# dsshim0125/s2p

Measured on AMD Instinct MI355X. Metric: G+D train-step images/sec at 84x84 bs=64/GPU, higher is better.
Workload: dtype bf16; 1 GPU; configs[2]: full G+D train step (hinge GAN + feature matching + VGG19 perceptual + L1, Adam x2), 84x84 cheetah, netG=s2p, netD=multiscale(2); global_batch=64, per_gpu_batch=64, parallelism=dp1, hip_graph=True, graph_segments=1, streams=overlapped, vgg_weights=seeded stand-in (ImageNet weights unobtainable offline)

## Files before the change

### include/s2p_hip.h

```cpp
#ifndef S2P_HIP_H
#define S2P_HIP_H
#include <stddef.h>
#include <stdint.h>

#ifdef __cplusplus
extern "C" {
#endif
#pragma GCC visibility push(default)

#define S2P_VERSION 125

enum { S2P_F32 = 0, S2P_BF16 = 1 };
enum { S2P_ACT_NONE = 0, S2P_ACT_RELU = 1, S2P_ACT_LRELU = 2, S2P_ACT_TANH = 3, S2P_ACT_SWISH = 4 };
enum { S2P_EPI_STORE = 0,
       S2P_EPI_ADD = 1,
       S2P_EPI_MUL_ACTGRAD = 2   };

typedef struct {
  int32_t dtype;
  int32_t N, H, W, Cin, x_pitch;
  int32_t Ho, Wo, Cout, y_pitch;
  int32_t KH, KW, stride, pad;
  int32_t transposed;
  int32_t reflect;
  int32_t groups;
  int32_t x_gstride, y_gstride;
  int32_t cin_real;
} s2p_conv_desc;

int s2p_version(void);
const char* s2p_last_error(void);

int s2p_conv2d_fwd(const s2p_conv_desc* d, const void* x, const void* w_fwd, const float* bias,
                   const void* aux, void* y, int act, float slope, int epi, void* stream);
int s2p_conv2d_dgrad(const s2p_conv_desc* d, const void* dy, const void* w_bwd,
                     const void* aux, const void* aux2, void* dx, int epi, int aux_act, float slope,
                     void* stream);
size_t s2p_conv2d_fwd_workspace(const s2p_conv_desc* d, int epi);
int s2p_conv2d_fwd_ws(const s2p_conv_desc* d, const void* x, const void* w_fwd, const float* bias,
                      const void* aux, void* y, int act, float slope, int epi, void* workspace,
                      size_t workspace_bytes, void* stream);
size_t s2p_conv2d_dgrad_workspace(const s2p_conv_desc* d);
int s2p_conv2d_dgrad_ws(const s2p_conv_desc* d, const void* dy, const void* w_bwd,
                        const void* aux, const void* aux2, void* dx, int epi, int aux_act, float slope,
                        void* workspace, size_t workspace_bytes, void* stream);
int s2p_conv2d_fwd_mat(const s2p_conv_desc* d, const void* x, const void* w_fwd, const float* bias, const void* aux,
                       void* y, int epi, const void* gb_img, int gb_pitch, const float* gb_st, int gb_st_pitch,
                       int act, float slope, float eps, void* y_mat, int y_mat_pitch, float* stats, void* workspace,
                       size_t workspace_bytes, void* stream);
int s2p_conv2d_dgrad_mat(const s2p_conv_desc* d, const void* dy, const void* w_bwd, void* d_mid, const void* aux, const void* xn,
                         int xn_pitch, const float* stats, const void* gb_img, int gb_pitch, const float* gb_st,
                         int gb_st_pitch, int act, float slope, float eps, float* sums, void* dxn, int dxn_pitch,
                         void* dgb_img, int dgb_pitch, float* dgb_st, int dgb_st_pitch, const void* res, int res_pitch,
                         void* workspace, size_t workspace_bytes, void* stream);
int s2p_conv2d_mat_is_fused(const s2p_conv_desc* d, int dgrad, int has_gb);
int s2p_conv2d_wgrad(const s2p_conv_desc* d, const void* x, const void* dy, float* dw, float* db,
                     int cin_real, int cout_real, int64_t dw_gstride, int splitk, void* stream);
size_t s2p_conv2d_wgrad_workspace(const s2p_conv_desc* d, int cin_real, int cout_real);
int s2p_conv2d_wgrad_ws(const s2p_conv_desc* d, const void* x, const void* dy, float* dw, float* db,
                        int cin_real, int cout_real, int64_t dw_gstride, int splitk, void* workspace,
                        size_t workspace_bytes, void* stream);
size_t s2p_conv2d_wgrad_det_workspace(const s2p_conv_desc* d, int cin_real, int cout_real, int splitk);
typedef struct { const void* x; const void* dy; float* dw; float* db; } s2p_wgrad_job;
size_t s2p_conv2d_wgrad_batched_workspace(const s2p_conv_desc* d, int n_jobs, int cin_real, int cout_real);
int s2p_conv2d_wgrad_batched(const s2p_conv_desc* d, const s2p_wgrad_job* jobs, int n_jobs, int cin_real,
                             int cout_real, void* workspace, size_t workspace_bytes, void* stream);
int s2p_reflect_pad_bwd(int dtype, const void* dxp, int N, int H, int W, int C, int pad, void* dx,
                        void* stream);
int s2p_channel_sum(int dtype, const void* dy, int64_t pixels, int C, int pitch, float* db,
                    void* stream);
size_t s2p_channel_sum_workspace(int64_t pixels, int C);
int s2p_channel_sum_ws(int dtype, const void* dy, int64_t pixels, int C, int pitch, float* db, void* workspace,
                       size_t workspace_bytes, void* stream);

int64_t s2p_in_stats_floats(int N, int HW, int C);
int s2p_in_stats(int dtype, const void* x, int N, int HW, int C, int pitch, float eps,
                 float* stats, void* stream);
int s2p_in_apply_fwd(int dtype, const void* x, int N, int HW, int C, int pitch,
                     const float* stats, const void* gb_img, int gb_pitch,
                     const float* gb_st, int gb_st_pitch, int act, float slope, float eps,
                     void* y, int y_pitch, void* stream);
int s2p_in_norm_fwd(int dtype, const void* x, int N, int HW, int C, int pitch, const void* gb_img, int gb_pitch,
                    const float* gb_st, int gb_st_pitch, int act, float slope, float eps, void* y, int y_pitch,
                    float* stats, void* stream);
int64_t s2p_in_bwd_sums_floats(int N, int HW, int C);
int s2p_in_bwd_reduce(int dtype, const void* da, int da_pitch, const void* x, int N, int HW, int C,
                      int pitch, const float* stats, const void* gb_img, int gb_pitch,
                      const float* gb_st, int gb_st_pitch, int act, float slope, float eps,
// ... 121 lines not shown
```

### s2p_amd/_lib.py

```python
import ctypes
import os
import subprocess

import torch

_HERE = os.path.dirname(os.path.abspath(__file__))
_SO = os.path.join(_HERE, "csrc", "libs2p_hip.so")

F32, BF16 = 0, 1
ACT_NONE, ACT_RELU, ACT_LRELU, ACT_TANH, ACT_SWISH = 0, 1, 2, 3, 4
EPI_STORE, EPI_ADD, EPI_MUL_ACTGRAD = 0, 1, 2

c_int, c_float, c_void_p, c_int64 = ctypes.c_int, ctypes.c_float, ctypes.c_void_p, ctypes.c_int64


class ConvDesc(ctypes.Structure):
    _fields_ = [(n, ctypes.c_int32) for n in (
        "dtype", "N", "H", "W", "Cin", "x_pitch", "Ho", "Wo", "Cout", "y_pitch",
        "KH", "KW", "stride", "pad", "transposed", "reflect", "groups", "x_gstride", "y_gstride", "cin_real")]


class L1Job(ctypes.Structure):
    _fields_ = [("a", c_void_p), ("b", c_void_p), ("grad_a", c_void_p), ("count", c_int64), ("scale", c_float),
                ("loss_out", c_void_p)]


class WgradJob(ctypes.Structure):
    _fields_ = [("x", c_void_p), ("dy", c_void_p), ("dw", c_void_p), ("db", c_void_p)]


class PackJob(ctypes.Structure):
    _fields_ = [("src", c_void_p), ("dst_fwd", c_void_p), ("dst_bwd", c_void_p),
                ("R", ctypes.c_int32), ("T", ctypes.c_int32), ("C", ctypes.c_int32),
                ("Cpad", ctypes.c_int32), ("Rrow", ctypes.c_int32), ("r_off", ctypes.c_int32),
                ("dtype", ctypes.c_int32)]


class SnJob(ctypes.Structure):
    _fields_ = [("w", c_void_p), ("u", c_void_p), ("v", c_void_p), ("sigma", c_void_p), ("ws", c_void_p), ("grad", c_void_p),
                ("R", ctypes.c_int32), ("K", ctypes.c_int32)]


_P = c_void_p
_DESC = ctypes.POINTER(ConvDesc)
SIGNATURES = {
    "s2p_version": [],
    "s2p_last_error": [],
    "s2p_conv2d_fwd": [_DESC, _P, _P, _P, _P, _P, c_int, c_float, c_int, _P],
    "s2p_conv2d_dgrad": [_DESC, _P, _P, _P, _P, _P, c_int, c_int, c_float, _P],
    "s2p_conv2d_fwd_workspace": [_DESC, c_int],
    "s2p_conv2d_fwd_ws": [_DESC, _P, _P, _P, _P, _P, c_int, c_float, c_int, _P, ctypes.c_size_t, _P],
    "s2p_conv2d_fwd_mat": [_DESC, _P, _P, _P, _P, _P, c_int, _P, c_int, _P, c_int, c_int, c_float, c_float, _P, c_int, _P, _P,
                           ctypes.c_size_t, _P],
    "s2p_conv2d_dgrad_mat": [_DESC, _P, _P, _P, _P, _P, c_int, _P, _P, c_int, _P, c_int, c_int, c_float, c_float, _P, _P, c_int, _P, c_int,
                             _P, c_int, _P, c_int, _P, ctypes.c_size_t, _P],
    "s2p_conv2d_mat_is_fused": [_DESC, c_int, c_int],
    "s2p_conv2d_dgrad_workspace": [_DESC],
    "s2p_conv2d_dgrad_ws": [_DESC, _P, _P, _P, _P, _P, c_int, c_int, c_float, _P, ctypes.c_size_t, _P],
    "s2p_conv2d_wgrad": [_DESC, _P, _P, _P, _P, c_int, c_int, c_int64, c_int, _P],
    "s2p_conv2d_wgrad_workspace": [_DESC, c_int, c_int],
    "s2p_conv2d_wgrad_det_workspace": [_DESC, c_int, c_int, c_int],
    "s2p_channel_sum_workspace": [c_int64, c_int],
    "s2p_channel_sum_ws": [c_int, _P, c_int64, c_int, c_int, _P, _P, ctypes.c_size_t, _P],
    "s2p_conv2d_wgrad_ws": [_DESC, _P, _P, _P, _P, c_int, c_int, c_int64, c_int, _P, ctypes.c_size_t, _P],
    "s2p_conv2d_wgrad_batched_workspace": [_DESC, c_int, c_int, c_int],
    "s2p_conv2d_wgrad_batched": [_DESC, ctypes.POINTER(WgradJob), c_int, c_int, c_int, _P, ctypes.c_size_t, _P],
    "s2p_reflect_pad_bwd": [c_int, _P, c_int, c_int, c_int, c_int, c_int, _P, _P],
    "s2p_channel_sum": [c_int, _P, c_int64, c_int, c_int, _P, _P],
    "s2p_in_stats": [c_int, _P, c_int, c_int, c_int, c_int, c_float, _P, _P],
    "s2p_in_apply_fwd": [c_int, _P, c_int, c_int, c_int, c_int, _P, _P, c_int, _P, c_int, c_int, c_float,
                         c_float, _P, c_int, _P],
    "s2p_in_norm_fwd": [c_int, _P, c_int, c_int, c_int, c_int, _P, c_int, _P, c_int, c_int, c_float, c_float, _P, c_int,
                        _P, _P],
    "s2p_in_bwd_reduce": [c_int, _P, c_int, _P, c_int, c_int, c_int, c_int, _P, _P, c_int, _P, c_int, c_int,
                          c_float, c_float, _P, _P],
    "s2p_in_bwd_apply": [c_int, _P, c_int, _P, c_int, c_int, c_int, c_int, _P, _P, c_int, _P, c_int, c_int,
                         c_float, c_float, _P, _P, c_int, _P, c_int, _P, c_int, _P],
    "s2p_in_norm_bwd": [c_int, _P, c_int, _P, c_int, c_int, c_int, c_int, _P, _P, c_int, _P, c_int, c_int,
                        c_float, c_float, _P, _P, c_int, _P, c_int, _P, c_int, _P],
    "s2p_in_norm_bwd_res": [c_int, _P, c_int, _P, c_int, c_int, c_int, c_int, _P, _P, c_int, _P, c_int, c_int,
                            c_float, c_float, _P, _P, c_int, _P, c_int, _P, c_int, _P, c_int, _P],
    "s2p_in_stats_floats": [c_int, c_int, c_int],
    "s2p_in_bwd_sums_floats": [c_int, c_int, c_int],
    "s2p_linear_fwd": [_P, c_int, c_int, c_int, _P, c_int, _P, c_int, c_int, c_float, _P, c_int, c_int, _P],
    "s2p_linear_bwd_workspace": [c_int, c_int, c_int],
    "s2p_linear_bwd": [_P, c_int, _P, c_int, _P, c_int, c_int, c_int, c_int, c_int, _P, c_int, c_int, c_float, _P, c_int, _P, _P,
                       c_int, _P, ctypes.c_size_t, _P],
    "s2p_gauss_head_fwd": [_P, c_int, c_int, c_int, _P, c_int, _P, c_int, _P, c_int, _P, c_int, _P, c_int, _P],
    "s2p_gauss_head_bwd": [_P, c_int, c_int, c_int, _P, c_int, _P, c_int, _P, c_int, _P, c_int, _P, c_int, _P, c_int, _P],
# ... 99 lines not shown
```

### s2p_amd/csrc/conv_igemm.hip

```cpp
#include "s2p_common.h"
#include "conv_plane.h"
#include "conv_planeg.h"
#include <type_traits>
#include <vector>

#define MAX_TAPS 64

constexpr int PHASE_TAPS = 16, MAX_PHASES = 4;
struct GatherArgs {
  const void* x; const void* w; const float* bias; const void* aux; const void* aux2; void* y;
  int M, Hi, Wi, Qh, Qw;
  int Cin, x_pitch, x_gstride;
  int Cout, Cst, y_pitch, y_gstride;
  int Ho, Wo;
  int istride, ostride, oy0, ox0;
  int T, Ktot, w_row;
  long long w_gstride;
  int reflect, act, epi, gact;
  float slope, gslope;
  int npix_tiles, nco_tiles;
  int halo_lo, halo_hi;
  int diag;
  int splitk, ksteps;
  float* part; int psplit, psteps, part_m;
  void* ws; size_t ws_bytes;
  size_t* plan; const PlaneMat* mat; int* mat_done;
  unsigned x_bytes, w_bytes;
  int tap[MAX_TAPS];
  int nphase, phase_fast;
  struct Phase { int Qh, Qw, M, oy0, ox0, T, Ktot, npix_tiles; int tap[PHASE_TAPS]; } ph[MAX_PHASES];
};

template <typename T> struct Mma;
template <> struct Mma<__bf16> { static constexpr int BK = 32; };
template <> struct Mma<float> { static constexpr int BK = 16; };
// ... 688 lines not shown
          if (aux2) x2.set(e, to_f32(aux2[go + e]));
        }
      }
#pragma unroll
      for (int e = 0; e < 8; ++e) {
        const float xv = x.get(e);
        const float f = g_tanh ? 1.f - xv * xv : (xv > 0.f ? 1.f : gneg);
        wv[e] = epi_add ? c.get(e) + xv : (c.get(e) + x2.get(e)) * f;
      }
      c.pack(wv);
    }
    if (full) *(u32x4*)(y + go) = c.raw;
    else for (int e = 0; e < 8; ++e) if (co0 + e < a.Cst) y[go + e] = from_f32<T>(c.get(e));
  }
}

struct ConvSwitches {
  int no_dma = s2p_env_set("S2P_NO_LDS_DMA");
  int diag = s2p_env_int("S2P_DIAG", 0);
  int no_halo = s2p_env_set("S2P_NO_HALO");
  int no_split = s2p_env_set("S2P_NO_CONV_SPLITK");
  int split_min_steps = s2p_env_int("S2P_SPLIT_MIN_STEPS", 16);
  int split_max_wg = s2p_env_int("S2P_SPLIT_MAX_WG", 160);
  int no_plane = s2p_env_set("S2P_NO_PLANE");
  int halo_extra_lds = s2p_env_int("S2P_HALO_EXTRA_LDS", 0);
  int no_static_taps = s2p_env_set("S2P_NO_STATIC_TAPS");
  int halo_pipe = s2p_env_set("S2P_NO_HALO_PIPE") ? 0 : 1;
  int no_merge = s2p_env_set("S2P_NO_PHASE_MERGE") || s2p_env_set("S2P_NO_LDS_DMA");
  int no_thin_cin = s2p_env_set("S2P_NO_THIN_CIN");
  static bool no_planeg() { return S2P_DIAG_SWITCH(0); }
  static bool no_planeg_3x3() { return S2P_DIAG_SWITCH(2); }
  static bool no_thin4() { return S2P_DIAG_SWITCH(3); }
  static bool no_phase_fast() { return S2P_DIAG_SWITCH(10); }
};
static const ConvSwitches& conv_switches() { static const ConvSwitches sw; return sw; }

static int conv_split_plan(int nwg, int nk) {
  const int min_steps = conv_switches().split_min_steps, max_wg = conv_switches().split_max_wg;
  if (nwg > max_wg || nk < 2 * min_steps) return 1;
  int S = 384 / nwg;
  if (S > nk / min_steps) S = nk / min_steps;
  if (S > 16) S = 16;
  return S < 2 ? 1 : S;
}

template <int NPOS_CAP, bool DBUF, int TS = 0, bool PIPE = false>
__global__ __launch_bounds__(256, 2) void conv_halo_kernel(const GatherArgs a) {
  typedef __bf16 T;
  constexpr int BCO = 128, BPIX = 128, WPIX = 2, TCO = 2, TPIX = 2;
  constexpr int BK = 64, RS = 128;
  constexpr int WSTAGE = BCO * RS;
  constexpr int HALO = (NPOS_CAP + 1) * RS;
  constexpr int ERS = BCO * 2 + 16;
  constexpr int EPI = BPIX * ERS;
  constexpr int NHB = DBUF ? 2 : 1;
  constexpr int MAIN0 = NHB * HALO + 2 * WSTAGE + 1024;
  constexpr int MAIN = MAIN0 > EPI ? MAIN0 : EPI;
  __shared__ __attribute__((aligned(1024))) char smem[MAIN + BPIX * 4];
  int* rowoff = (int*)(smem + MAIN);
  char* hbase = smem;
  char* wbase = smem + NHB * HALO;
  char* zrow = smem + NHB * HALO + 2 * WSTAGE;
  unsigned long long tl0 = 0, tl1 = 0, tl2 = 0;
  if (S2P_DIAGV(a) == 9) tl0 = __builtin_amdgcn_s_memrealtime();

  const int tid = threadIdx.x;
// ... 361 lines not shown
#pragma unroll
      for (int s = 0; s < 4; ++s)
#pragma unroll
        for (int i = 0; i < TCO; ++i)
#pragma unroll
          for (int j = 0; j < TPIX; ++j)
            acc[i][j] = __builtin_amdgcn_mfma_f32_32x32x16_bf16(af[s][i], bf[s][j], acc[i][j], 0, 0, 0);
    }
    __syncthreads();
    tap = ntap;
    tw_cur = tw_next; tw_next = tw_next2;
    if (nslab_i != slab) {
      slab = nslab_i;
      if (!DBUF && slab < nslab) {
        issue_halo(0, slab * BK);
        __syncthreads();
      }
    }
  }
  (void)nk;
  if (S2P_DIAGV(a) == 8) {
    const unsigned long long c1 = __builtin_amdgcn_s_memtime(), r1 = __builtin_amdgcn_s_memrealtime();
    if (tid == 0 && g == 0) {
      unsigned long long* o = (unsigned long long*)a.y + (size_t)blockIdx.x * 2;
      o[0] = c1 - st_c0; o[1] = r1 - st_r0;
    }
    if (acc[0][0][0] == 12345.678f) ((float*)a.y)[7] = acc[1][1][3] + acc[0][1][2] + acc[1][0][1];
    return;
  }
  if (S2P_DIAGV(a) == 4) { if (acc[0][0][0] == 12345.678f) ((float*)a.y)[0] = acc[1][1][3] + acc[0][1][2] + acc[1][0][1]; return; }
  conv_epilogue<T, BCO, BPIX, TCO, TPIX>(a, acc, smem, rowoff, g, co_base, wco0, wpix0, r, h, tid);
}

enum class ConvPath { Thin, Thin4, ThinCin, ThinRows, Plane, PlaneG, Halo, SplitK, Dma, Fast, Phases, Generic };
enum class HaloKind { S9_176_PIPE, S9_176, S9_320, R_176, R_320 };

struct ConvOperands {
  const void* x; const void* w; const float* bias; const void* aux; const void* aux2; void* y;
  int act; float slope; int epi, gact; float gslope;
};
struct NormWant { bool any, gb, bwd; };
struct ScratchAvail { bool any; size_t bytes; };
static const ScratchAvail SCRATCH_UNLIMITED{true, ~(size_t)0};
struct Scratch { void* ws; size_t bytes; };

struct GatherChoice {
  ConvPath path = ConvPath::Generic;
  bool fused = false;
  size_t ws_bytes = 0;
  int bco = 128;
  HaloKind halo = HaloKind::R_320;
  PlaneArgs plane;
  PlaneGArgs planeg;
};
struct GatherItem { GatherArgs a; GatherChoice c; };
struct ConvPlan {
  ConvPath path = ConvPath::Generic;
  bool fused = false;
  size_t ws_bytes = 0;
  int cout_pad = 0;
  std::vector<GatherItem> items;
  void add(const GatherItem& it) {
    if (items.empty()) path = it.c.path;
    if (it.c.ws_bytes > ws_bytes) ws_bytes = it.c.ws_bytes;
    items.push_back(it);
    fused = items.size() == 1 && it.c.fused;
  }
};

template <typename P>
static void copy_conv_fields(P& p, const GatherArgs& a) {
  p.x = a.x; p.w = a.w; p.bias = a.bias; p.aux = a.aux; p.aux2 = a.aux2; p.y = a.y;
  p.Cin = a.Cin; p.x_pitch = a.x_pitch; p.x_gstride = a.x_gstride;
  p.Cout = a.Cout; p.Cst = a.Cst; p.y_pitch = a.y_pitch; p.y_gstride = a.y_gstride;
  p.w_row = a.w_row; p.w_gstride = a.w_gstride;
  p.act = a.act; p.epi = a.epi; p.gact = a.gact; p.slope = a.slope; p.gslope = a.gslope;
  p.x_bytes = a.x_bytes; p.w_bytes = a.w_bytes;
}
template <typename P>
static void copy_norm(P& p, const PlaneMat& m) {
  p.xn = m.xn; p.xn_pitch = m.xn_pitch; p.dgb = m.dgb; p.dgb_pitch = m.dgb_pitch;
  p.dgbst = m.dgbst; p.dgbst_pitch = m.dgbst_pitch; p.res = m.res; p.res_pitch = m.res_pitch;
  p.y2 = m.y2; p.y2_pitch = m.y2_pitch; p.gb = m.gb; p.gb_pitch = m.gb_pitch;
  p.gbst = m.gbst; p.gbst_pitch = m.gbst_pitch; p.stats = m.stats;
  p.n_act = m.act; p.n_slope = m.slope; p.eps = m.eps;
}
// ... 121 lines not shown
  a.T = G.KH * G.KW; a.Ktot = a.T * G.Ci; a.reflect = G.reflect;
  if (a.T > MAX_TAPS) S2P_FAIL(-2, "conv: more than %d taps", MAX_TAPS);
  for (int ky = 0; ky < G.KH; ++ky)
    for (int kx = 0; kx < G.KW; ++kx) a.tap[ky * G.KW + kx] = pack_tap(ky - G.pad, kx - G.pad, ky * G.KW + kx);
  if (a.M > 0) P.add(plan_gather(a, bf16, G.groups, gathered_elems(G), want, sc));
  return 0;
}

static int plan_scatter_problem(const Geo& G, bool bf16, const ConvOperands& op, const NormWant& want, const ScratchAvail& sc, ConvPlan& P) {
  const ConvSwitches& sw = conv_switches();
  const int s = G.stride;
  GatherArgs base = gather_base(G, op);
  base.istride = 1; base.ostride = s;
  const long long xb = gathered_elems(G) * 2, wb = (long long)G.Co * G.w_row * 2;
  if (bf16 && !sw.no_merge && s * s <= MAX_PHASES && s > 1 && G.Ci % 64 == 0 && xb < (1ll << 31) && wb < (1ll << 31) && G.Cst > 32) {
    GatherItem it{base, {}};
    GatherArgs& a = it.a;
    a.x_bytes = (unsigned)xb; a.w_bytes = (unsigned)wb;
    a.diag = sw.diag;
    bool ok = true;
    int np = 0;
    for (int py = 0; py < s && ok; ++py)
      for (int px = 0; px < s && ok; ++px) {
        GatherArgs::Phase& ph = a.ph[np];
        ph.Qh = (G.Ho - py + s - 1) / s; ph.Qw = (G.Wo - px + s - 1) / s;
        if (ph.Qh <= 0 || ph.Qw <= 0) continue;
        ph.M = G.N * ph.Qh * ph.Qw; ph.oy0 = py; ph.ox0 = px;
        ph.T = phase_taps(G, py, px, ph.tap, PHASE_TAPS);
        if (ph.T <= 0) { ok = false; break; }
        ph.Ktot = ph.T * G.Ci;
        ph.npix_tiles = cdiv(ph.M, 128);
        ++np;
      }
    if (ok && np > 0) {
      a.nphase = np;
      it.c.path = ConvPath::Phases;
      it.c.bco = a.Cst > 64 ? 128 : 64;
      a.nco_tiles = cdiv(a.Cst, it.c.bco);
      a.phase_fast = (it.c.bco == 64 && !sw.no_phase_fast()) ? 1 : 0;
      P.add(it);
      return 0;
    }
  }
  for (int py = 0; py < s; ++py)
    for (int px = 0; px < s; ++px) {
      GatherArgs a = base;
      a.Qh = (G.Ho - py + s - 1) / s; a.Qw = (G.Wo - px + s - 1) / s;
      if (a.Qh <= 0 || a.Qw <= 0) continue;
      a.M = G.N * a.Qh * a.Qw; a.oy0 = py; a.ox0 = px;
      a.T = phase_taps(G, py, px, a.tap, MAX_TAPS);
      if (a.T < 0) S2P_FAIL(-2, "conv: more than %d taps", MAX_TAPS);
      a.Ktot = a.T * G.Ci;
      if (a.M > 0) P.add(plan_gather(a, bf16, G.groups, gathered_elems(G), want, sc));
    }
  return 0;
}

static int check_desc(const s2p_conv_desc* d, const char* who) {
  if (!d) S2P_FAIL(-1, "%s: null desc", who);
  if (d->dtype != S2P_F32 && d->dtype != S2P_BF16) S2P_FAIL(-1, "%s: bad dtype %d", who, d->dtype);
  int ce = d->dtype == S2P_F32 ? 4 : 8;
  if (d->Cin % ce || d->x_pitch % ce || d->y_pitch % ce || d->x_gstride % ce || d->y_gstride % ce)
    S2P_FAIL(-1, "%s: Cin/pitches must be multiples of %d elements (Cin=%d xp=%d yp=%d)", who, ce, d->Cin,
             d->x_pitch, d->y_pitch);
  if (d->groups < 1 || d->stride < 1 || d->KH < 1 || d->KW < 1) S2P_FAIL(-1, "%s: bad geometry", who);
  if (d->x_pitch < d->Cin || d->y_pitch < d->Cout) S2P_FAIL(-1, "%s: pitch smaller than channels", who);
// ... 79 lines not shown
    default:
      hipLaunchKernelGGL((conv_dma_kernel<BCO, 128, 2, 2>), grid, dim3(256), 0, st, a);
      S2P_CHECK_LAUNCH("conv_dma_kernel");
      return 0;
  }
}

template <typename T>
static int launch_generic(GatherArgs& a, int groups, hipStream_t st) {
  if (a.Cst > 64) return launch_cfg<T, 128, 128, 2, 2>(a, groups, st);
  if (a.Cst > 32) return launch_cfg<T, 64, 128, 2, 2>(a, groups, st);
  return launch_cfg<T, 32, 256, 1, 4>(a, groups, st);
}

static int launch_item(GatherItem& it, bool bf16, int groups, const PlaneMat* mat, void* ws, hipStream_t st) {
  if (!bf16) return launch_generic<float>(it.a, groups, st);
  switch (it.c.path) {
    case ConvPath::Plane:
      if (it.c.fused) copy_norm(it.c.plane, *mat);
      return s2p_conv_plane_launch(it.c.plane, groups, st);
    case ConvPath::PlaneG:
      if (it.c.fused) copy_norm(it.c.planeg, *mat);
      return s2p_conv_planeg_launch(it.c.planeg, groups, st);
    case ConvPath::Phases: {
      GatherArgs& a = it.a;
      int max_npt = 0;
      for (int i = 0; i < a.nphase; ++i) if (a.ph[i].npix_tiles > max_npt) max_npt = a.ph[i].npix_tiles;
      const dim3 grid = a.phase_fast ? dim3(((max_npt * a.nco_tiles + 7) / 8) * 8 * a.nphase, groups, 1) : dim3(max_npt * a.nco_tiles, groups, a.nphase);
      if (it.c.bco == 128) hipLaunchKernelGGL((conv_dma_kernel<128, 128, 2, 2>), grid, dim3(256), 0, st, a);
      else hipLaunchKernelGGL((conv_dma_kernel<64, 128, 2, 2>), grid, dim3(256), 0, st, a);
      S2P_CHECK_LAUNCH("conv_dma_kernel(phases)");
      return 0;
    }
    case ConvPath::Generic: break;
    default: return it.c.bco == 128 ? launch_bf16<128>(it.a, it.c, groups, ws, st) : launch_bf16<64>(it.a, it.c, groups, ws, st);
  }
  return launch_generic<__bf16>(it.a, groups, st);
}
static int launch_items(ConvPlan& P, bool bf16, int groups, const PlaneMat* mat, const Scratch& sc, hipStream_t st) {
  for (GatherItem& it : P.items) {
    const int rc = launch_item(it, bf16, groups, mat, sc.ws, st);
    if (rc) return rc;
  }
  return 0;
}

static int conv_fwd_impl(const s2p_conv_desc* d, const ConvOperands& op, const PlaneMat* mat, bool* fused, const Scratch& sc, void* stream) {
  S2P_CHECK_SLOPE("s2p_conv2d_fwd", op.act, op.slope);
  if (mat) S2P_CHECK_SLOPE("s2p_conv2d_fwd_mat", mat->act, mat->slope);
  ConvPlan P;
  int rc = conv_plan_fwd(d, op, NormWant{mat != nullptr, mat && mat->gb, false}, ScratchAvail{sc.ws != nullptr, sc.bytes}, P);
  if (rc) return rc;
  if (!op.x || !op.w || (!op.y && !mat)) S2P_FAIL(-1, "s2p_conv2d_fwd: null pointer");
  if (op.epi != S2P_EPI_STORE && !op.aux) S2P_FAIL(-1, "s2p_conv2d_fwd: epi needs aux");
  if (!op.y && !P.fused) S2P_FAIL(-1, "s2p_conv2d_fwd_mat: y == NULL needs the fused launch (s2p_conv2d_mat_is_fused)");
  if (fused) *fused = P.fused;
  hipStream_t st = (hipStream_t)stream;
  switch (P.path) {
    case ConvPath::Thin: return s2p_thin_fwd(d, op.x, op.w, op.bias, op.y, op.act, op.slope, st);
    case ConvPath::Thin4: return s2p_thin4_fwd(d, op.x, op.w, op.bias, op.y, op.act, op.slope, sc.ws, sc.bytes, st);
    case ConvPath::ThinCin: return s2p_thin_cin_fwd(d, op.x, op.w, op.bias, op.y, op.act, op.slope, st);
    default: return launch_items(P, d->dtype == S2P_BF16, d->groups, mat, sc, st);
  }
}

extern "C" int s2p_conv2d_fwd(const s2p_conv_desc* d, const void* x, const void* w_fwd, const float* bias,
// ... 62 lines not shown
                                    int xn_pitch, const float* stats, const void* gb_img, int gb_pitch, const float* gb_st,
                                    int gb_st_pitch, int act, float slope, float eps, float* sums, void* dxn, int dxn_pitch,
                                    void* dgb_img, int dgb_pitch, float* dgb_st, int dgb_st_pitch, const void* res, int res_pitch,
                                    void* workspace, size_t workspace_bytes, void* stream) {
  if (!d || !xn || !stats || !dxn) S2P_FAIL(-1, "s2p_conv2d_dgrad_mat: null pointer");
  if (act != S2P_ACT_NONE && act != S2P_ACT_RELU && act != S2P_ACT_LRELU) S2P_FAIL(-1, "s2p_conv2d_dgrad_mat: activation must be none / relu / lrelu");
  if (d->groups != 1 || d->transposed || d->reflect) S2P_FAIL(-1, "s2p_conv2d_dgrad_mat: groups == 1, not transposed, zero padding");
  if (d->Cin != d->x_pitch) S2P_FAIL(-1, "s2p_conv2d_dgrad_mat: the produced tensor must be dense (x_pitch %d != Cin %d)", d->x_pitch, d->Cin);
  PlaneMat m{dxn, dxn_pitch, gb_img, gb_pitch, gb_st, gb_st_pitch, const_cast<float*>(stats), act, slope, eps,
             xn, xn_pitch, dgb_img, dgb_pitch, dgb_st, dgb_st_pitch, res, res_pitch};
  bool fused = false;
  int rc = conv_dgrad_impl(d, ConvOperands{dy, w_bwd, nullptr, aux, nullptr, d_mid ? d_mid : dxn, S2P_ACT_NONE, 0.f,
                                           aux ? S2P_EPI_ADD : S2P_EPI_STORE, S2P_ACT_NONE, 0.f},
                           &m, !d_mid || !sums, &fused, Scratch{workspace, workspace_bytes}, stream);
  if (rc || fused) return rc;
  return s2p_in_norm_bwd_res(d->dtype, d_mid, d->x_pitch, xn, d->N, d->H * d->W, d->Cin, xn_pitch, stats, gb_img, gb_pitch, gb_st,
                             gb_st_pitch, act, slope, eps, sums, dxn, dxn_pitch, dgb_img, dgb_pitch, dgb_st, dgb_st_pitch, res,
                             res_pitch, stream);
}
extern "C" int s2p_conv2d_mat_is_fused(const s2p_conv_desc* d, int dgrad, int has_gb) {
  if (!d || d->groups != 1 || d->transposed || d->reflect) return 0;
  const ConvOperands op{nullptr, nullptr, nullptr, nullptr, nullptr, nullptr, S2P_ACT_NONE, 0.f, S2P_EPI_STORE, S2P_ACT_NONE, 0.f};
  const NormWant want{true, has_gb != 0, dgrad != 0};
  ConvPlan P;
  const int rc = dgrad ? conv_plan_dgrad(d, op, want, SCRATCH_UNLIMITED, P) : conv_plan_fwd(d, op, want, SCRATCH_UNLIMITED, P);
  return rc == 0 && P.fused ? 1 : 0;
}
extern "C" size_t s2p_conv2d_dgrad_workspace(const s2p_conv_desc* d) {
  ConvPlan P;
  if (conv_plan_dgrad(d, ConvOperands{nullptr, nullptr, nullptr, nullptr, nullptr, nullptr, S2P_ACT_NONE, 0.f, S2P_EPI_STORE, S2P_ACT_NONE, 0.f},
                      NormWant{}, SCRATCH_UNLIMITED, P)) return 0;
  return P.ws_bytes;
}
```

Measured before the change: 7666 images/sec.

## Add sub-pixel fused kernel for stride-2 transposed conv phases

Adds a specialized kernel that computes all four output phases of a stride-2, 3x3-style transposed convolution in a single block. It loads one shared input halo per channel slab and reuses it across the nine weight taps, instead of running each phase as a separate gather tile. This is meant to cut redundant input loads and launch/tile overhead for the generator's upsampling convs. The cost is a more complex kernel with a 4-slot weight ring and double-buffered halo, and the path only applies to restricted shapes (Cin multiple of 64, Cst 64 or 128, narrow width).

```diff
diff --git a/include/s2p_hip.h b/include/s2p_hip.h
--- a/include/s2p_hip.h
+++ b/include/s2p_hip.h
@@ -54,6 +54,9 @@
                          void* dgb_img, int dgb_pitch, float* dgb_st, int dgb_st_pitch, const void* res, int res_pitch,
                          void* workspace, size_t workspace_bytes, void* stream);
 int s2p_conv2d_mat_is_fused(const s2p_conv_desc* d, int dgrad, int has_gb);
+enum { S2P_CONV_PATH_PHASES = 10, S2P_CONV_PATH_SUBPIXEL = 12 };
+int s2p_conv2d_plan_path(const s2p_conv_desc* d, int dgrad, int epi);
+int s2p_conv2d_subpixel_enable(int on);
 int s2p_conv2d_wgrad(const s2p_conv_desc* d, const void* x, const void* dy, float* dw, float* db,
                      int cin_real, int cout_real, int64_t dw_gstride, int splitk, void* stream);
 size_t s2p_conv2d_wgrad_workspace(const s2p_conv_desc* d, int cin_real, int cout_real);
diff --git a/s2p_amd/_lib.py b/s2p_amd/_lib.py
--- a/s2p_amd/_lib.py
+++ b/s2p_amd/_lib.py
@@ -55,6 +55,8 @@
     "s2p_conv2d_dgrad_mat": [_DESC, _P, _P, _P, _P, _P, c_int, _P, _P, c_int, _P, c_int, c_int, c_float, c_float, _P, _P, c_int, _P, c_int,
                              _P, c_int, _P, c_int, _P, ctypes.c_size_t, _P],
     "s2p_conv2d_mat_is_fused": [_DESC, c_int, c_int],
+    "s2p_conv2d_plan_path": [_DESC, c_int, c_int],
+    "s2p_conv2d_subpixel_enable": [c_int],
     "s2p_conv2d_dgrad_workspace": [_DESC],
     "s2p_conv2d_dgrad_ws": [_DESC, _P, _P, _P, _P, _P, c_int, c_int, c_float, _P, ctypes.c_size_t, _P],
     "s2p_conv2d_wgrad": [_DESC, _P, _P, _P, _P, c_int, c_int, c_int64, c_int, _P],
diff --git a/s2p_amd/csrc/conv_igemm.hip b/s2p_amd/csrc/conv_igemm.hip
--- a/s2p_amd/csrc/conv_igemm.hip
+++ b/s2p_amd/csrc/conv_igemm.hip
@@ -1,6 +1,7 @@
 #include "s2p_common.h"
 #include "conv_plane.h"
 #include "conv_planeg.h"
+#include "conv_subpixel.h"
 #include <type_traits>
 #include <vector>
 
@@ -755,6 +756,8 @@
   static bool no_planeg_3x3() { return S2P_DIAG_SWITCH(2); }
   static bool no_thin4() { return S2P_DIAG_SWITCH(3); }
   static bool no_phase_fast() { return S2P_DIAG_SWITCH(10); }
+  static bool no_subpixel() { return subpixel_off() != 0 || S2P_DIAG_SWITCH(21); }
+  static int& subpixel_off() { static int off = 0; return off; }
 };
 static const ConvSwitches& conv_switches() { static const ConvSwitches sw; return sw; }
 
@@ -1182,7 +1185,8 @@
   conv_epilogue<T, BCO, BPIX, TCO, TPIX>(a, acc, smem, rowoff, g, co_base, wco0, wpix0, r, h, tid);
 }
 
-enum class ConvPath { Thin, Thin4, ThinCin, ThinRows, Plane, PlaneG, Halo, SplitK, Dma, Fast, Phases, Generic };
+enum class ConvPath { Thin, Thin4, ThinCin, ThinRows, Plane, PlaneG, Halo, SplitK, Dma, Fast, Phases, Generic, SubPixel };
+static_assert((int)ConvPath::Phases == S2P_CONV_PATH_PHASES && (int)ConvPath::SubPixel == S2P_CONV_PATH_SUBPIXEL, "s2p_conv2d_plan_path ids (s2p_hip.h)");
 enum class HaloKind { S9_176_PIPE, S9_176, S9_320, R_176, R_320 };
 
 struct ConvOperands {
@@ -1202,6 +1206,7 @@
   HaloKind halo = HaloKind::R_320;
   PlaneArgs plane;
   PlaneGArgs planeg;
+  SubPixelArgs subpixel;
 };
 struct GatherItem { GatherArgs a; GatherChoice c; };
 struct ConvPlan {
@@ -1389,6 +1394,16 @@
         ph.npix_tiles = cdiv(ph.M, 128);
         ++np;
       }
+    if (ok && np > 0 && !ConvSwitches::no_subpixel()) {
+      SubPixelProblem pr{G.N, G.Hi, G.Wi, G.Ho, G.Wo, G.Ci, G.Co, G.Cst, s, G.groups, np, {}};
+      for (int i = 0; i < np && i < 4; ++i) pr.ph[i] = {a.ph[i].oy0, a.ph[i].ox0, a.ph[i].T, a.ph[i].tap};
+      if (s2p_conv_subpixel_setup(pr, it.c.subpixel)) {
+        copy_conv_fields(it.c.subpixel, a);
+        it.c.path = ConvPath::SubPixel;
+        P.add(it);
+        return 0;
+      }
+    }
     if (ok && np > 0) {
       a.nphase = np;
       it.c.path = ConvPath::Phases;
@@ -1534,6 +1549,7 @@
       S2P_CHECK_LAUNCH("conv_dma_kernel(phases)");
       return 0;
     }
+    case ConvPath::SubPixel: return s2p_conv_subpixel_launch(it.c.subpixel, st);
     case ConvPath::Generic: break;
     default: return it.c.bco == 128 ? launch_bf16<128>(it.a, it.c, groups, ws, st) : launch_bf16<64>(it.a, it.c, groups, ws, st);
   }
@@ -1662,3 +1678,15 @@
                       NormWant{}, SCRATCH_UNLIMITED, P)) return 0;
   return P.ws_bytes;
 }
+
+extern "C" int s2p_conv2d_plan_path(const s2p_conv_desc* d, int dgrad, int epi) {
+  const ConvOperands op{nullptr, nullptr, nullptr, nullptr, nullptr, nullptr, S2P_ACT_NONE, 0.f, epi, S2P_ACT_NONE, 0.f};
+  ConvPlan P;
+  const int rc = dgrad ? conv_plan_dgrad(d, op, NormWant{}, SCRATCH_UNLIMITED, P) : conv_plan_fwd(d, op, NormWant{}, SCRATCH_UNLIMITED, P);
+  return rc ? -1 : (int)P.path;
+}
+extern "C" int s2p_conv2d_subpixel_enable(int on) {
+  const int was = ConvSwitches::subpixel_off() ? 0 : 1;
+  ConvSwitches::subpixel_off() = on ? 0 : 1;
+  return was;
+}
diff --git a/s2p_amd/csrc/conv_subpixel.h b/s2p_amd/csrc/conv_subpixel.h
--- /dev/null
+++ b/s2p_amd/csrc/conv_subpixel.h
@@ -0,0 +1,24 @@
+#pragma once
+#include <hip/hip_runtime.h>
+
+struct SubPixelArgs {
+  const void* x; const void* w; const float* bias; const void* aux; const void* aux2; void* y;
+  int N, Hi, Wi, Ho, Wo;
+  int M;
+  int Cin, x_pitch, x_gstride;
+  int Cout, Cst, y_pitch, y_gstride;
+  int w_row;
+  long long w_gstride;
+  int act, epi, gact;
+  float slope, gslope;
+  unsigned x_bytes, w_bytes;
+  int wt[9];
+  int npix_tiles, nco_tiles;
+};
+
+struct SubPixelProblem {
+  int N, Hi, Wi, Ho, Wo, Cin, Cout, Cst, stride, groups, nphase;
+  struct Ph { int py, px, T; const int* tap; } ph[4];
+};
+bool s2p_conv_subpixel_setup(const SubPixelProblem& p, SubPixelArgs& a);
+int s2p_conv_subpixel_launch(const SubPixelArgs& a, hipStream_t st);
diff --git a/s2p_amd/csrc/conv_subpixel.hip b/s2p_amd/csrc/conv_subpixel.hip
--- /dev/null
+++ b/s2p_amd/csrc/conv_subpixel.hip
@@ -0,0 +1,293 @@
+#include "s2p_common.h"
+#include "conv_subpixel.h"
+
+namespace {
+constexpr int SP_BPIX = 128, SP_BCO = 64, SP_RS = 128;
+constexpr int SP_NPOS = 176;
+constexpr int SP_NPIECE = SP_NPOS / 8;
+constexpr int SP_NHP = (SP_NPIECE + 3) / 4;
+constexpr int SP_HALO = (SP_NPOS + 1) * SP_RS;
+constexpr int SP_WST = SP_BCO * SP_RS;
+constexpr int SP_RING = 4;
+constexpr int SP_MAIN = 2 * SP_HALO + SP_RING * SP_WST;
+constexpr int SP_ERS = SP_BCO * 2 + 16;
+constexpr int SP_EPX = SP_BPIX * SP_ERS + 128;
+static_assert(2 * SP_EPX <= SP_MAIN, "epilogue tile must fit the staging area");
+constexpr int SP_STEPS = 9;
+__host__ __device__ constexpr int sp_sh(int u) { return u < 4 ? 0 : (u < 6 ? 1 : (u < 8 ? 2 : 3)); }
+__host__ __device__ constexpr int sp_ph(int u) { return u < 4 ? u : (u == 4 ? 1 : (u == 6 ? 2 : 3)); }
+
+__global__ __launch_bounds__(256, 2) void conv_subpixel_kernel(const SubPixelArgs a) {
+  typedef __bf16 T;
+  __shared__ __attribute__((aligned(1024))) char smem[SP_MAIN + 4 * SP_BPIX * 4];
+  int* rowoff = (int*)(smem + SP_MAIN);
+  char* hbase = smem;
+  char* wbase = smem + 2 * SP_HALO;
+
+  const int tid = threadIdx.x;
+  const int lane = tid & 63;
+  const int wave = __builtin_amdgcn_readfirstlane(tid >> 6);
+  const int r = lane & 31, h = lane >> 5;
+  const int nblk = a.npix_tiles * a.nco_tiles;
+  int bid = blockIdx.x;
+  {
+    const int q8 = nblk >> 3, r8 = nblk & 7, xcd = bid & 7, k = bid >> 3;
+    bid = (xcd < r8 ? xcd * (q8 + 1) : r8 * (q8 + 1) + (xcd - r8) * q8) + k;
+  }
+  const int co_tile = bid % a.nco_tiles, pix_tile = bid / a.nco_tiles;
+  const int co_base = co_tile * SP_BCO, pix_base = pix_tile * SP_BPIX;
+  const int HW = a.Hi * a.Wi;
+  const double rcpHW = s2p_rcp_f64(HW), rcpW = s2p_rcp_f64(a.Wi);
+  auto split_pixel = [&](int m, int& n, int& qy, int& qx) {
+    int rr;
+    n = divmod_rcp(m, HW, rcpHW, rr);
+    qy = divmod_rcp(rr, a.Wi, rcpW, qx);
+  };
+  for (int e = tid; e < 4 * SP_BPIX; e += 256) {
+    const int py = e >> 8, px = e & 1, m = pix_base + ((e & 255) >> 1);
+    int off = -1;
+    if (m < a.M) {
+      int n, qy, qx;
+      split_pixel(m, n, qy, qx);
+      const int oy = 2 * qy + py, ox = 2 * qx + px;
+      if (oy < a.Ho && ox < a.Wo) off = (n * a.Ho + oy) * a.Wo + ox;
+    }
+    rowoff[e] = off;
+  }
+  if (tid < 16) *(u32x4*)(hbase + (tid >> 3) * SP_HALO + SP_NPOS * SP_RS + (tid & 7) * 16) = (u32x4){0u, 0u, 0u, 0u};
+  __syncthreads();
+
+  const unsigned OOB = 0x80000000u;
+  const i32x4 wrs = s2p_make_rsrc(a.w, a.w_bytes);
+  const i32x4 xrs = s2p_make_rsrc(a.x, a.x_bytes);
+  const unsigned wb_lds = __builtin_amdgcn_readfirstlane(s2p_lds_addr(wbase));
+  const unsigned hb_lds = __builtin_amdgcn_readfirstlane(s2p_lds_addr(hbase));
+  const int lrow = lane >> 3, pc = lane & 7;
+  unsigned wv[2];
+#pragma unroll
+  for (int q = 0; q < 2; ++q) {
+    const int row = (wave + 4 * q) * 8 + lrow;
+    const int c = pc ^ ((row >> 1) & 7);
+    const int co = co_base + row;
+    wv[q] = co < a.Cout ? (unsigned)(co * a.w_row * 2 + c * 16) : OOB;
+  }
+  unsigned hv[SP_NHP]; int hpc[SP_NHP];
+#pragma unroll
+  for (int i = 0; i < SP_NHP; ++i) {
+    int pc8 = 4 * i + wave;
+    if (pc8 >= SP_NPIECE) pc8 -= 4;
+    hpc[i] = pc8;
+    const int pos = pc8 * 8 + lrow;
+    const int c = pc ^ ((pos >> 1) & 7);
+    const long long gpix = (long long)pix_base + pos;
+    hv[i] = gpix < a.M ? (unsigned)(gpix * a.x_pitch * 2 + c * 16) : OOB;
+  }
+  int wtv[SP_STEPS];
+#pragma unroll
+  for (int u = 0; u < SP_STEPS; ++u) wtv[u] = a.wt[u];
+  auto issue_w = [&](int slot, int wt, int kofs, bool valid) {
+    const unsigned dst = wb_lds + (unsigned)(slot * SP_WST + wave * 1024);
+    const unsigned woff = (unsigned)((wt * a.Cin + kofs) * 2);
+#pragma unroll
+    for (int q = 0; q < 2; ++q)
+      s2p_dma16(wrs, dst + q * 4096, (int)((wv[q] == OOB || !valid) ? OOB : wv[q] + woff));
+  };
+  auto issue_halo = [&](int hbuf, int c0) {
+    const unsigned dst = hb_lds + (unsigned)(hbuf * SP_HALO);
+#pragma unroll
+    for (int i = 0; i < SP_NHP; ++i)
+      s2p_dma16(xrs, dst + (unsigned)(hpc[i] * 1024), (int)(hv[i] == OOB ? OOB : hv[i] + (unsigned)(c0 * 2)));
+  };
+
+  const int wco0 = (wave >> 1) * 32, wpix0 = (wave & 1) * 64;
+  const int arow = (wco0 + r) * SP_RS, swr = (r >> 1) & 7;
+  const int ch16[4] = {(0 + h) * 16, (2 + h) * 16, (4 + h) * 16, (6 + h) * 16};
+  int pk[4][2];
+#pragma unroll
+  for (int j = 0; j < 2; ++j) {
+    const int p = wpix0 + 32 * j + r, m = pix_base + p;
+    int n = 0, qy = a.Hi, qx = a.Wi;
+    if (m < a.M) split_pixel(m, n, qy, qx);
+#pragma unroll
+    for (int sh = 0; sh < 4; ++sh) {
+      const int dy = sh >> 1, dx = sh & 1;
+      const int hp = p + dy * a.Wi + dx;
+      const bool ok = qy + dy < a.Hi && qx + dx < a.Wi;
+      pk[sh][j] = ok ? hp * SP_RS + ((hp >> 1) & 7) * 16 : SP_NPOS * SP_RS;
+    }
+  }
+
+  f32x16 acc[4][2];
+#pragma unroll
+  for (int p = 0; p < 4; ++p)
+#pragma unroll
+    for (int j = 0; j < 2; ++j)
+#pragma unroll
+      for (int e = 0; e < 16; ++e) acc[p][j][e] = 0.f;
+
+  const int nslab = a.Cin / 64;
+  issue_halo(0, 0);
+  issue_w(0, wtv[0], 0, true);
+  issue_w(1, wtv[1], 0, true);
+  issue_w(2, wtv[2], 0, true);
+  S2P_WAIT_VMCNT(4);
+  __builtin_amdgcn_s_barrier();
+  __builtin_amdgcn_sched_barrier(0);
+  int hs = 0;
+  bf16x8 FB[4][2];
+  for (int slab = 0; slab < nslab; ++slab) {
+    const char* hb = hbase + (slab & 1) * SP_HALO;
+    const bool more = slab + 1 < nslab;
+    s2p_static_for<0, SP_STEPS>([&](auto uc) {
+      constexpr int u = decltype(uc)::value;
+      constexpr int u3 = (u + 3) % SP_STEPS;
+      constexpr bool wrap = u + 3 >= SP_STEPS;
+      issue_w((hs + 3) & 3, wtv[u3], (slab + (wrap ? 1 : 0)) * 64, wrap ? more : true);
+      if constexpr (u == 0) {
+        if (more) issue_halo((slab + 1) & 1, (slab + 1) * 64);
+      }
+      if constexpr (u == 0 || sp_sh(u) != sp_sh(u > 0 ? u - 1 : 0)) {
+#pragma unroll
+        for (int s = 0; s < 4; ++s)
+#pragma unroll
+          for (int j = 0; j < 2; ++j) FB[s][j] = *(const bf16x8*)(hb + (pk[sp_sh(u)][j] ^ ch16[s]));
+      }
+      const char* wst = wbase + (hs & 3) * SP_WST + arow;
+      bf16x8 FA[4];
+#pragma unroll
+      for (int s = 0; s < 4; ++s) FA[s] = *(const bf16x8*)(wst + (((2 * s + h) ^ swr) * 16));
+#pragma unroll
+      for (int s = 0; s < 4; ++s)
+#pragma unroll
+        for (int j = 0; j < 2; ++j)
+          acc[sp_ph(u)][j] = __builtin_amdgcn_mfma_f32_32x32x16_bf16(FA[s], FB[s][j], acc[sp_ph(u)][j], 0, 0, 0);
+      if (u < 3 && more) S2P_WAIT_VMCNT(4 + SP_NHP); else S2P_WAIT_VMCNT(4);
+      __builtin_amdgcn_s_barrier();
+      __builtin_amdgcn_sched_barrier(0);
+      ++hs;
+    });
+  }
+  S2P_WAIT_VMCNT(0);
+  __syncthreads();
+
+  const bool act_generic = (a.act == S2P_ACT_TANH || a.act == S2P_ACT_SWISH);
+  const float ns = a.act == S2P_ACT_RELU ? 0.f : (a.act == S2P_ACT_LRELU ? a.slope : 1.f);
+  if (a.bias) {
+    const __amdgpu_buffer_rsrc_t brs = __builtin_amdgcn_make_buffer_rsrc((void*)a.bias, 0, a.Cout * 4, 0x00020000);
+#pragma unroll
+    for (int q4 = 0; q4 < 4; ++q4) {
+      const int co = co_base + wco0 + 8 * q4 + 4 * h;
+      float bv[4];
+#pragma unroll
+      for (int e = 0; e < 4; ++e) bv[e] = __builtin_bit_cast(float, __builtin_amdgcn_raw_buffer_load_b32(brs, co * 4, e * 4, 0));
+#pragma unroll
+      for (int p = 0; p < 4; ++p)
+#pragma unroll
+        for (int j = 0; j < 2; ++j)
+#pragma unroll
+          for (int e = 0; e < 4; ++e) acc[p][j][4 * q4 + e] += bv[e];
+    }
+  }
+  if (act_generic) {
+#pragma unroll
+    for (int p = 0; p < 4; ++p)
+#pragma unroll
+      for (int j = 0; j < 2; ++j)
+#pragma unroll
+        for (int e = 0; e < 16; ++e) {
+          const float t = acc[p][j][e];
+          acc[p][j][e] = a.act == S2P_ACT_TANH ? tanhf(t) : t / (1.f + expf(-t));
+        }
+  }
+  T* yg = (T*)a.y;
+  const T* auxg = (const T*)a.aux;
+  const T* aux2g = (const T*)a.aux2;
+  const bool epi_add = a.epi == S2P_EPI_ADD;
+  const bool g_tanh = a.gact == S2P_ACT_TANH;
+  const float gneg = a.gact == S2P_ACT_RELU ? 0.f : (a.gact == S2P_ACT_LRELU ? a.gslope : 1.f);
+#pragma unroll
+  for (int py = 0; py < 2; ++py) {
+    if (py) __syncthreads();
+#pragma unroll
+    for (int px = 0; px < 2; ++px)
+#pragma unroll
+      for (int q4 = 0; q4 < 4; ++q4) {
+        const int col = wco0 + 8 * q4 + 4 * h;
+#pragma unroll
+        for (int j = 0; j < 2; ++j) {
+          char* dst = smem + px * SP_EPX + (wpix0 + 32 * j + r) * SP_ERS + col * 2;
+          float v[4];
+#pragma unroll
+          for (int e = 0; e < 4; ++e) {
+            const float t = acc[py * 2 + px][j][4 * q4 + e];
+            v[e] = act_generic ? t : lrelu_ns(t, ns);
+          }
+          const bf16x4 o = {(__bf16)v[0], (__bf16)v[1], (__bf16)v[2], (__bf16)v[3]};
+          *(bf16x4*)dst = o;
+        }
+      }
+    __syncthreads();
+    for (int idx = tid; idx < 2 * SP_BPIX * 8; idx += 256) {
+      const int row = idx >> 3, ch = idx & 7;
+      const int off = rowoff[py * 2 * SP_BPIX + row];
+      if (off < 0) continue;
+      const int co0 = co_base + ch * 8;
+      Chunk<T> c;
+      c.raw = *(const u32x4*)(smem + (row & 1) * SP_EPX + (row >> 1) * SP_ERS + ch * 16);
+      const size_t go = (size_t)off * a.y_pitch + co0;
+      if (a.epi != S2P_EPI_STORE) {
+        Chunk<T> x, x2;
+        x2.raw = (u32x4){0u, 0u, 0u, 0u};
+        x.raw = *(const u32x4*)(auxg + go);
+        if (aux2g) x2.raw = *(const u32x4*)(aux2g + go);
+        float ov[8];
+#pragma unroll
+        for (int e = 0; e < 8; ++e) {
+          const float v = c.get(e), xv = x.get(e);
+          const float f = g_tanh ? 1.f - xv * xv : (xv > 0.f ? 1.f : gneg);
+          ov[e] = epi_add ? v + xv : (v + x2.get(e)) * f;
+        }
+        c.pack(ov);
+      }
+      *(u32x4*)(yg + go) = c.raw;
+    }
+  }
+}
+}
+
+bool s2p_conv_subpixel_setup(const SubPixelProblem& p, SubPixelArgs& a) {
+  if (p.stride != 2 || p.groups != 1 || p.nphase != 4) return false;
+  if (p.Cin % 64 != 0 || !(p.Cst == 64 || p.Cst == 128)) return false;
+  if (SP_BPIX + p.Wi + 1 > SP_NPOS) return false;
+  if (p.Ho > 2 * p.Hi || p.Wo > 2 * p.Wi) return false;
+  if ((long long)p.N * p.Ho * p.Wo >= (1ll << 31)) return false;
+  int wtab[4][4];
+  for (int s = 0; s < 4; ++s) for (int q = 0; q < 4; ++q) wtab[s][q] = -1;
+  for (int q = 0; q < 4; ++q) {
+    if (p.ph[q].py * 2 + p.ph[q].px != q) return false;
+    for (int t = 0; t < p.ph[q].T; ++t) {
+      const int ti = p.ph[q].tap[t];
+      const int dy = (int)(signed char)(ti & 0xff), dx = (int)(signed char)((ti >> 8) & 0xff);
+      if (dy < 0 || dy > 1 || dx < 0 || dx > 1 || wtab[dy * 2 + dx][q] >= 0) return false;
+      wtab[dy * 2 + dx][q] = ti >> 16;
+    }
+  }
+  int nz = 0;
+  for (int s = 0; s < 4; ++s) for (int q = 0; q < 4; ++q) nz += wtab[s][q] >= 0;
+  if (nz != SP_STEPS) return false;
+  for (int u = 0; u < SP_STEPS; ++u) {
+    if (wtab[sp_sh(u)][sp_ph(u)] < 0) return false;
+    a.wt[u] = wtab[sp_sh(u)][sp_ph(u)];
+  }
+  a.N = p.N; a.Hi = p.Hi; a.Wi = p.Wi; a.Ho = p.Ho; a.Wo = p.Wo;
+  a.M = p.N * p.Hi * p.Wi;
+  a.npix_tiles = (a.M + SP_BPIX - 1) / SP_BPIX;
+  a.nco_tiles = p.Cst / SP_BCO;
+  return a.M > 0;
+}
+
+int s2p_conv_subpixel_launch(const SubPixelArgs& a, hipStream_t st) {
+  hipLaunchKernelGGL(conv_subpixel_kernel, dim3(a.npix_tiles * a.nco_tiles), dim3(256), 0, st, a);
+  S2P_CHECK_LAUNCH("conv_subpixel_kernel");
+  return 0;
+}
```

New measurement: 7713 images/sec (median of 6 runs). About the same (+0.6%).
